# bderembl/msom

Hardware: AMD Instinct MI355X
Metric: grid-point-updates/s (timesteps/s x N^2 x nl), multi-layer QG RK2 step at 4096x4096x6 per GPU (higher is better)
Workload: dtype f64; 1 GPU; C4: msqg double gyre (Verron 1992 params), 4096x4096x6 fp64, tiles 1x1 of 4096x4096, TOLERANCE 1e-3, RK2 step = 2 inversions + 2 tendencies + 2 advances; mg_nrelax=4

## Files before the change

msom_amd/csrc/kernels.h:

```cpp
#ifndef MSOM_KERNELS_H
#define MSOM_KERNELS_H

#include <stdio.h>
#include <stdlib.h>

#include <type_traits>
#include <utility>

#include "msom_internal.h"
#include "modes_inl.h"
#include "floats_inl.h"

template <int LO, int HI, class F>
static inline bool with_int(int v, F &&f) {
  if constexpr (LO > HI) return false;
  else {
    if (v == LO) { f(std::integral_constant<int, LO>{}); return true; }
    return with_int<LO + 1, HI>(v, std::forward<F>(f));
  }
}
template <class F>
static inline void with_bool(bool b, F &&f) {
  if (b) f(std::true_type{});
  else f(std::false_type{});
// ... 180 lines not shown
                        const SplitGeom &sg, int nl, const RelaxCoef &rc, int walls, int nh, int c0, const double *S = nullptr);
void launch_relax_block2(hipStream_t st, const KernelOpts &o, const double *da_in, const double *coarse, const SplitGeom &cg, const double *res, double *da_out,
                         const SplitGeom &sg, int nl, const RelaxCoef &rc, int walls, int fine);
void launch_relax_red_prolong(hipStream_t st, const KernelOpts &o, double *da, const double *coarse, const SplitGeom &cg, const double *res, const double *S,
                              const SplitGeom &sg, int nl, const RelaxCoef &rc, int uniformS, int walls);
void launch_correct(hipStream_t st, double *a, const NatGeom &g, const double *da, const SplitGeom &sg, int nl, int walls);

struct VisitRingBands { int s0[4], ns[4], c0[4], nc[4], n; };
struct MarchCorrect { const double *psi; double *psi_out; NatGeom g; };
struct MarchHalo { const double *in_s, *in_n, *res_s, *res_n; size_t ls; int rows; };
int launch_relax_march(hipStream_t st, const KernelOpts &o, const double *in, double *out, const double *res, const SplitGeom &sg, int nl, const RelaxCoef &rc, int c1,
                       int K, int walls, int chunk_rows = 0, const MarchHalo *h = nullptr, const double *coarse = nullptr, const SplitGeom *cg = nullptr,
                       const MarchCorrect *mc = nullptr, int more_follow = 0, const MarchHalo *coarse_halo = nullptr, int region = 0,
                       const int *skip = nullptr, int skip_compact = 0);
int launch_relax_visit(hipStream_t st, const KernelOpts &o, double *da, double *da_alt, const double *res, const SplitGeom &sg, int nl, const RelaxCoef &rc,
                       int walls, const double *coarse, const SplitGeom &cg, const MarchCorrect &mc);
bool relax_visit_fits(int nl, const SplitGeom &sg, int rows, int pairs);
extern "C" int msom_visit_ring(int hk, int ny, int march_rows, int visit_rows, int pairs, int corr, int *geom, int *bands);
bool march_lean_fits(int nl, const SplitGeom &sg, const NatGeom *ng);

struct ModeCoef {
  double m2l[MSOM_MAXNL * MSOM_MAXNL], ibu[MSOM_MAXNL];
};
int launch_modes_eig(hipStream_t st, const double *S, const NatGeom &g, int nl, int ncx, int ncy, double *out, size_t ols, int per_column,
                     const ModesLayers &l, int *flag);
int launch_modes_get(hipStream_t st, double *out, const double *md, const ModeCoef *mc, const NatGeom &g, int nl, const ModesLayers &l, int which,
                     int first, int cnt);
int launch_modes_rd(hipStream_t st, double *rd, const double *md, const ModeCoef *mc, const NatGeom &g, int nl, int mode);
int launch_modes_project(hipStream_t st, const double *in, double *out, const double *md, const ModeCoef *mc, const NatGeom &g, int nl,
                         const ModesLayers &l, int to_modes);
int modes_energy_blocks(const NatGeom &g);
int modes_energy_stride(const NatGeom &g);
// ... 146 lines not shown
```

msom_amd/csrc/kernels_march.hip:

```cpp
#include <algorithm>
#include <map>
#include <mutex>
#include <type_traits>
#include <utility>
#include "mg_inl.h"
#include "rhs_inl.h"

#pragma clang fp contract(off)

__device__ __forceinline__ double march_rhs(double sqD, double rs, double we, double ns) {
#ifdef MSOM_STRICT
  double v = -sqD * rs;
  v += we;
  v += ns;
  return v;
#else
  return fma(-sqD, rs, we) + ns;
#endif
}
template <int NL>
__device__ __forceinline__ void march_thomas(double (&rhs)[NL], double (&x)[NL], const RelaxCoef &rc) {
#ifdef MSOM_STRICT
#pragma unroll
  for (int l = 1; l < NL; l++) rhs[l] -= rc.w[l] * rhs[l - 1];
// ... 251 lines not shown
            nat_write_ghosts(p.psi_out, p.ng, l, r, 2 * kx, ve, p.walls);
            nat_write_ghosts(p.psi_out, p.ng, l, r, 2 * kx + 1, vo, p.walls);
          }
        }
      }
    }
  }
}

template <int NL, int K, int HL, int WPB, bool PL, bool CORR, int VIS = 0>
struct MarchLeanRows {
  static constexpr int NLE = (NL + 1) & ~1;
  static constexpr int CB = 2 * NLE;
  static constexpr int PBL = (VIS == 2 ? 2 : 3) * NLE;
  static constexpr int XBL = PBL + 2 * NL;
  static constexpr int ROWS = PL ? CB + 4 * NLE : (CORR ? XBL + NL : 3 * NLE);
  static constexpr int RB = PL ? 2 * NLE : 3 * NLE;
  static constexpr int CBD = 2 * RB;
  static constexpr int ROWSD = PL ? CBD + 2 * NLE : 2 * RB;
};

#define MARCH_VMCNT(N) asm volatile("s_waitcnt vmcnt(%0)" ::"n"(N) : "memory")
typedef double v2d __attribute__((ext_vector_type(2)));

template <int NL, int K, int HL, int WPB, bool PL, bool CORR, bool DEEP, int VIS = 0>
__device__ __forceinline__ void march_lean(const MarchArgs &p, double (*ring)[64], const int lane, const int kx0, const int y0, const int y1,
                                           const bool down, double (*hand)[64] = nullptr) {
  static_assert(VIS == 0 || (VIS == 1 && PL && !CORR) || (VIS == 2 && CORR), "fused visit: prolongation leads, correction trails");
  using LR = MarchLeanRows<NL, K, HL, WPB, PL, CORR, VIS>;
  constexpr int D1 = K >= 3 ? 3 : 1, D2 = K >= 4 ? 3 : 1;
  static_assert(!(DEEP && CORR), "no LDS for a second buffer beside the psi block");
  constexpr int NLE = LR::NLE, ND = NLE / 2, CB = DEEP ? LR::CBD : LR::CB, PBL = LR::PBL, XBL = LR::XBL, RB = LR::RB;
  constexpr int CSLOTS = DEEP ? 2 : 4;
  constexpr int NREQ = (PL ? 2 : 3) * ND;
  const int kx = kx0 + lane;
  const bool own_lane = lane >= HL && lane < 64 - HL;
  const int d = down ? -1 : 1;
  const long long rp8 = (long long)p.g.rp * 8, hp8 = (long long)p.g.hp * 8, ls8 = (long long)p.g.ls * 8;
  const long long drp8 = down ? -rp8 : rp8;
  const double sqD = p.rc.sqD;
  const unsigned lds0 = __builtin_amdgcn_readfirstlane((unsigned)(unsigned long long)(__attribute__((address_space(3))) double *)(&ring[0][0]));
  const int sub = lane >> 5;
  unsigned voffL[ND];
// ... 10 lines not shown
      const int la = 2 * q + sub < NL ? 2 * q + sub : NL - 1;
      voffC[q] = (unsigned)(((size_t)la * p.cg.ls + ((lane >> 4) & 1) * p.cg.hp + MSOM_SP + (kx0 >> 1) + 2 * (lane & 15)) * 8);
    }
  }
  const int cld = (lane & 1) * 32 + (lane >> 1);
  const long long crp8 = (long long)p.cg.rp * 8;
  const unsigned voffN = (unsigned)((MSOM_XP + 2 * kx) * 8);
  const long long np8 = (long long)p.ng.pitch * 8, nls8 = (long long)p.ng.ls * 8;
  const long long dnp8 = down ? -np8 : np8;

  const int tA = y0 - K + 1, tB = y1 + K - 2;
  int ra = down ? y0 + y1 - 1 - tA : tA;
  long long rowoff = ((long long)(ra + 1) * p.g.rp + ((ra + p.c1) & 1) * p.g.hp) * 8;
  const char *const res8 = reinterpret_cast<const char *>(p.res);
  const char *const resb8 = res8 - drp8;
  const char *const in8 = PL ? nullptr : reinterpret_cast<const char *>(p.in) + drp8;
  char *const outK8 = CORR ? nullptr : reinterpret_cast<char *>(p.out) - (long long)(K - 1) * drp8;
  long long natoff = CORR ? ((long long)(ra - d * K + MSOM_YP) * p.ng.pitch) * 8 : 0;
  const char *const psi8 = reinterpret_cast<const char *>(p.psi);
  char *const pso8 = reinterpret_cast<char *>(p.psi_out);
  const char *const co8 = reinterpret_cast<const char *>(p.coarse);

  unsigned m0keep;
#define MARCH_DMA(voff, base, ldsrow) \
  asm volatile("s_mov_b32 m0, %2\n\ts_nop 3\n\tglobal_load_lds_dwordx4 %0, %1" ::"v"(voff), "s"(base), "s"(lds0 + (unsigned)(ldsrow) * 512u) : "memory")
  auto request = [&](long long ro, long long no, bool want_psi, int buf = 0) {
    asm volatile("s_mov_b32 %0, m0" : "=s"(m0keep));
    const char *b1 = res8 + ro, *b2 = resb8 + ro;
    const int r0 = buf * RB;
#pragma unroll
    for (int q = 0; q < ND; q++) MARCH_DMA(voffL[q], b1, r0 + 2 * q);
// ... 725 lines not shown
  a.hls = h ? h->ls : 0; a.KR = h ? h->rows : 0;
  a.lean = !o.march_lean ? 0 : o.march_lean * (int)(march_lean_fits(nl, sg, mc ? &mc->g : nullptr) && (!coarse || c1 == 0));
  a.in = in; a.out = out; a.res = res; a.g = sg; a.c1 = c1; a.walls = walls; a.rc = rc; a.remap = o.march_xcd; a.flip = o.march_flip; a.dbg = o.march_dbg;
  if (nl >= 7 && K > 3) return -1;
  int r = -1;
  with_int<1, MSOM_FASTNL>(nl, [&](auto N) { r = march_dispatch<N()>(st, a, K, chunk_rows, o.march_dma); });
  return r;
}

__device__ __forceinline__ void xcd_remap_lin(const unsigned lin, const unsigned nbx, const unsigned total, unsigned &bx, unsigned &by) {
  const unsigned c = lin & 7, q = total >> 3, r = total & 7;
  const unsigned flat = c * q + (c < r ? c : r) + (lin >> 3);
  bx = flat % nbx;
  by = flat / nbx;
}
template <int NL, int PAIRS, int VIS, int KIND>
__device__ __forceinline__ void visit_role(const MarchArgs &p, double (*lds)[64], const int pair) {
  constexpr int K = 4, HL = 8;
  constexpr int OW = 64 - 2 * HL;
  constexpr int RA = MarchLeanRows<NL, K, HL, 2, true, false>::ROWSD, RB = MarchLeanRows<NL, K, HL, 2, false, true, 2>::ROWS;
  const int lane = threadIdx.x & 63;
  unsigned bx = blockIdx.x, by = blockIdx.y;
  if constexpr (KIND != 0) {
    const unsigned lin = blockIdx.x - (unsigned)p.ring_wg;
    if (p.remap) xcd_remap_lin(lin, p.fnbx, (unsigned)p.fnbx * p.fnby, bx, by);
    else { bx = lin % (unsigned)p.fnbx; by = lin / (unsigned)p.fnbx; }
    by += p.fby0;
  } else {
    if (p.remap) xcd_remap(bx, by);
  }
  const int kx0 = p.vx0 + ((int)bx * PAIRS + pair) * OW - HL;
  const int y0 = p.vy0 + (int)by * p.H, y1 = y0 + p.H;
  const bool down = p.flip && (by & 1);
  double(*ring)[64] = lds + pair * (RA + RB + 2 * NL);
  double(*hand)[64] = ring + RA + RB;
  if constexpr (VIS == 2) march_lean<NL, K, HL, 2, false, true, false, 2>(p, ring + RA, lane, kx0, y0, y1, down, hand);
  else march_lean<NL, K, HL, 2, true, false, true, 1>(p, ring, lane, kx0, y0 - K, y1 + K, down, hand);
}
template <int NL, int KIND>
__device__ __forceinline__ void visit_ring_role(const MarchArgs &p, double (*lds)[64], const int wv, const int nwv) {
  constexpr int K = 4;
  const int i = (int)blockIdx.x * nwv + wv;
  if (i >= p.rb.n) return;
  int strip;
  unsigned by;
  visit_ring_chunk(p.rb, i, strip, by);
  MarchArgs q = p;
  q.H = p.rH; q.lean = p.rlean; q.in = p.rin; q.out = p.rout;
  q.partial = KIND == 1;
  q.rb.n = 0; q.region = 0; q.sy0 = q.sy1 = 0;
  const int lane = threadIdx.x & 63;
  if constexpr (KIND == 1) march_dma_chunk<NL, K, 4, 1, true, false>(q, lds + wv * MarchDmaRows<NL, K, 4, 1, true, false>::LROWS, lane, strip, by);
  else march_dma_chunk<NL, K, 2, 1, false, true>(q, lds + wv * MarchDmaRows<NL, K, 2, 1, false, true>::LROWS, lane, strip, by);
}
template <int NL, int PAIRS, int KIND>
__global__ void __launch_bounds__(128 * PAIRS, 2) k_relax_visit(MarchArgs p) {
  constexpr int K = 4, HL = 8;
  constexpr int RA = MarchLeanRows<NL, K, HL, 2, true, false>::ROWSD, RB = MarchLeanRows<NL, K, HL, 2, false, true, 2>::ROWS;
  constexpr int RPL = MarchDmaRows<NL, K, 4, 1, true, false>::LROWS, RCO = MarchDmaRows<NL, K, 2, 1, false, true>::LROWS;
  constexpr int RFUSED = PAIRS * (RA + RB + 2 * NL), RRING = KIND == 0 ? 0 : 2 * PAIRS * (KIND == 1 ? RPL : RCO);
  __shared__ __align__(16) double lds[RFUSED > RRING ? RFUSED : RRING][64];
  const int wv = __builtin_amdgcn_readfirstlane((int)(threadIdx.x >> 6));
  if constexpr (KIND != 0) {
    if ((int)blockIdx.x < p.ring_wg) {
      visit_ring_role<NL, KIND>(p, lds, wv, 2 * PAIRS);
      return;
    }
  }
  if (wv & 1) visit_role<NL, PAIRS, 2, KIND>(p, lds, wv >> 1);
  else visit_role<NL, PAIRS, 1, KIND>(p, lds, wv >> 1);
}

struct VisitGeom { int H, vy0, nc, vx0, ns; };
static bool visit_geom(int hk, int ny, int rows, int pairs, VisitGeom &v) {
  constexpr int K = 4, HL = 8, OW = 64 - 2 * HL;
  v.H = rows > 0 ? (rows + 1) & ~1 : 28;
  v.vy0 = 2 * K;
  v.nc = (ny - 2 * K - v.vy0) / v.H;
  v.vx0 = HL;
  v.ns = hk >= 64 ? ((hk - 64) / OW + 1) / pairs * pairs : 0;
  return v.nc > 0 && v.ns > 0;
}
bool relax_visit_fits(int nl, const SplitGeom &sg, int rows, int pairs) {
  VisitGeom v;
  return nl >= 2 && nl <= 6 && (pairs == 1 || pairs == 2) && visit_geom(sg.hk, sg.ny, rows, pairs, v);
}

static void visit_ring_bands(int hk, int ny, int ow, int H, const int *skip, VisitRingBands &rb) {
  const int ns = (hk + ow - 1) / ow, nc = (ny + H - 1) / H;
  int s_lo = std::min(ns, (std::max(skip[2], 0) + ow - 1) / ow), s_hi = hk <= skip[3] ? ns : std::max(skip[3], 0) / ow;
  int c_lo = std::min(nc, (std::max(skip[0], 0) + H - 1) / H), c_hi = ny <= skip[1] ? nc : std::max(skip[1], 0) / H;
  if (skip[1] <= skip[0] || s_lo >= s_hi || c_lo >= c_hi) { c_lo = c_hi = nc; s_lo = s_hi = ns; }
  const int s0[4] = {0, 0, 0, s_hi}, n_s[4] = {ns, ns, s_lo, ns - s_hi}, c0[4] = {0, c_hi, c_lo, c_lo}, n_c[4] = {c_lo, nc - c_hi, c_hi - c_lo, c_hi - c_lo};
  rb.n = 0;
  for (int b = 0; b < 4; b++) {
    rb.s0[b] = s0[b]; rb.ns[b] = n_s[b]; rb.c0[b] = c0[b]; rb.nc[b] = n_c[b];
    rb.n += n_s[b] * n_c[b];
  }
}
static void visit_skips(const VisitGeom &v, int Hc, int *skip_pl, int *skip_corr) {
// ... 7 lines not shown
extern "C" int msom_visit_ring(int hk, int ny, int march_rows, int visit_rows, int pairs, int corr, int *geom, int *bands) {
  VisitGeom v;
  if (hk <= 0 || ny <= 0 || (pairs != 1 && pairs != 2) || !visit_geom(hk, ny, visit_rows, pairs, v)) return -1;
  int skip_pl[4], skip_corr[4];
  const int Hc = visit_ring_rows(march_rows);
  visit_skips(v, Hc, skip_pl, skip_corr);
  VisitRingBands rb;
  visit_ring_bands(hk, ny, corr ? 60 : 56, Hc, corr ? skip_corr : skip_pl, rb);
  if (geom) { geom[0] = v.H; geom[1] = v.vy0; geom[2] = v.nc; geom[3] = v.vx0; geom[4] = v.ns; }
  if (bands)
    for (int b = 0; b < 4; b++) { bands[b] = rb.s0[b]; bands[4 + b] = rb.ns[b]; bands[8 + b] = rb.c0[b]; bands[12 + b] = rb.nc[b]; }
  return rb.n;
}

template <int NL>
static void visit_dispatch(hipStream_t st, const MarchArgs &a, const VisitGeom &v, int pairs) {
  const dim3 grid = a.ring_kind ? dim3(a.ring_wg + a.fnbx * a.fnby) : dim3(v.ns / pairs, v.nc);
  with_int<0, 2>(a.ring_kind, [&](auto R) {
    with_int<1, 2>(pairs, [&](auto P) {
      constexpr int PAIRS = decltype(P)::value;
      hipLaunchKernelGGL((k_relax_visit<NL, PAIRS, decltype(R)::value>), grid, dim3(128 * PAIRS), 0, st, a);
    });
  });
}
static void visit_dispatch_nl(hipStream_t st, const MarchArgs &a, const VisitGeom &v, int pairs, int nl) {
  if (!with_int<2, 6>(nl, [&](auto N) { visit_dispatch<N()>(st, a, v, pairs); })) no_kernel("launch_relax_visit", nl);
}

int launch_relax_visit(hipStream_t st, const KernelOpts &o, double *da, double *da_alt, const double *res, const SplitGeom &sg, int nl, const RelaxCoef &rc,
                       int walls, const double *coarse, const SplitGeom &cg, const MarchCorrect &mc) {
  const int rows = o.march_visit_rows, pairs = o.march_visit_pairs;
  VisitGeom v;
  if (!relax_visit_fits(nl, sg, rows, pairs)) return -1;
  visit_geom(sg.hk, sg.ny, rows, pairs, v);
  constexpr int K = 4;
  const int Hc = visit_ring_rows(o.march_rows);
  int skip_pl[4], skip_corr[4];
  visit_skips(v, Hc, skip_pl, skip_corr);
  if (o.march_dbg & 16) {
    for (int *s : {skip_pl, skip_corr}) { s[0] = 0; s[1] = sg.ny; s[2] = 0; s[3] = sg.hk; }
  }
  const int ringopt = o.march_visit_ring;
  MarchArgs a{};
  a.res = res; a.g = sg; a.c1 = 0; a.walls = walls; a.rc = rc;
  a.coarse = coarse; a.cg = cg;
  a.psi = mc.psi; a.psi_out = mc.psi_out; a.ng = mc.g;
  a.partial = 1; a.lean = 2;
  a.remap = o.march_xcd; a.flip = o.march_flip;
  a.H = v.H; a.vy0 = v.vy0; a.vx0 = v.vx0;
  if (ringopt >= 2) {
    const int nwv = 2 * pairs;
    a.fnbx = v.ns / pairs;
    a.rH = Hc;
    a.rlean = o.march_lean ? o.march_lean * (int)march_lean_fits(nl, sg, &mc.g) : 0;
    const int n1 = std::min(v.nc, (o.march_visit_split > 0 ? o.march_visit_split : v.nc / 3)) & ~1;
    a.ring_kind = 1;
    visit_ring_bands(sg.hk, sg.ny, 56, Hc, skip_pl, a.rb);
    a.ring_wg = (a.rb.n + nwv - 1) / nwv;
    a.fby0 = 0; a.fnby = n1;
    a.rin = nullptr; a.rout = da_alt;
    visit_dispatch_nl(st, a, v, pairs, nl);
    a.ring_kind = 2;
    visit_ring_bands(sg.hk, sg.ny, 60, Hc, skip_corr, a.rb);
    a.ring_wg = (a.rb.n + nwv - 1) / nwv;
    a.fby0 = n1; a.fnby = v.nc - n1;
    a.rin = da_alt; a.rout = da;
    visit_dispatch_nl(st, a, v, pairs, nl);
    return 0;
  }
  if (launch_relax_march(st, o, nullptr, da_alt, res, sg, nl, rc, 0, K, walls, Hc, nullptr, coarse, &cg, nullptr, 1, nullptr, 0, skip_pl, ringopt == 1)) return -1;
  visit_dispatch_nl(st, a, v, pairs, nl);
  return launch_relax_march(st, o, da_alt, da, res, sg, nl, rc, 0, K, walls, Hc, nullptr, nullptr, nullptr, &mc, 0, nullptr, 0, skip_corr, ringopt == 1);
}
```

msom_amd/csrc/msom_api.hip:

```cpp
#include "msom_host.h"
#include "step_dt_inl.h"

#define RHS_RESID_MIN 23
#define RHS_CLOSE_MIN 23
#define RHS_CLOSE_DEFAULT 2
#define MARCH_HALO 4

static void free_agglomeration(msom *m);

extern "C" const char *msom_version(void) {
#ifdef MSOM_STRICT
  return "msomhip 0.1 (strict: -ffp-contract=off, reference expression order, bit-exact vs oracle)";
#else
  return "msomhip 0.1 (fast: FMA contraction, reciprocal multiplies)";
#endif
}


NatGeom make_nat(int nx, int ny) {
  NatGeom g;
  g.nx = nx; g.ny = ny;
  g.pitch = ((nx + 15) / 16) * 16 + 2 * MSOM_XP;
  g.rows = ny + 2 * MSOM_YP;
  g.ls = (size_t)g.pitch * g.rows;
// ... 456 lines not shown
  else if (!strcmp(key, "uniform_S")) {
    m->uniform_opt = (int)v;
    if (m->const_set) return build_coefs(m);
  }
  else if (!strcmp(key, "profile")) m->profile = (int)v;
  else if (!strcmp(key, "fused")) m->fused = (int)v;
  else if (!strcmp(key, "mg_fused")) m->mg_fused = (int)v;
  else if (!strcmp(key, "march")) m->march = (int)v;
  else if (!strcmp(key, "march_min")) m->march_min = (int)v;
  else if (!strcmp(key, "march_min_tiled")) m->march_min_tiled = (int)v;
  else if (!strcmp(key, "march_partial")) m->march_partial = (int)v;
  else if (!strcmp(key, "march_prolong")) m->march_prolong = (int)v;
  else if (!strcmp(key, "march_correct")) m->march_correct = (int)v;
  else if (!strcmp(key, "march_visit")) m->march_visit = (int)v;
  else if (!strcmp(key, "march_visit_min")) m->march_visit_min = (int)v;
  else if (!strcmp(key, "dbg_nosync")) m->dbg_nosync = (int)v;
  else if (!strcmp(key, "async_solve")) m->async_solve = (int)v;
  else if (!strcmp(key, "step_sync")) m->step_sync = (int)v;
  else if (!strcmp(key, "march_k")) m->march_k = (int)v < 2 ? 2 : ((int)v > 4 ? 4 : (int)v);
  else if (!strcmp(key, "block_small")) m->block_small = (int)v;
  else if (!strcmp(key, "block8")) m->block8 = (int)v;
  else if (!strcmp(key, "restrict2")) m->restrict2 = (int)v;
  else if (!strcmp(key, "restrict_pyr")) m->restrict_pyr = (int)v;
  else if (!strcmp(key, "block8_max")) m->block8_max = (int)v;
  else if (!strcmp(key, "block_sweeps")) { m->block_sweeps = (int)v; if (m->const_set) return build_coefs(m); }
  else if (!strcmp(key, "mg_global_sum")) m->mg_global_sum = (int)v;
  else if (!strcmp(key, "agglomerate")) { m->agglomerate = (int)v; if (m->const_set) return build_coefs(m); }
  else if (!strcmp(key, "agg_size")) { m->agg_size = (int)v; if (m->const_set) return build_coefs(m); }
  else if (!strcmp(key, "prolong_fused")) { m->prolong_fused = (int)v; if (m->const_set) return build_coefs(m); }
  else if (!strcmp(key, "mg_coarse")) { m->mgc_opt = (int)v; if (m->const_set) return build_coefs(m); }
// ... 50 lines not shown
        HIPCHK(hipMalloc(&m->f[k], bytes));
        HIPCHK(hipMemsetAsync(m->f[k], 0, bytes, m->st));
      }
    }
  } else {
    msom_set_error("unknown option %s", key);
    return MSOM_ERR_ARG;
  }
  return MSOM_OK;
}

static int march_levels(const msom *m);
static int march_kmax(const msom *m);
static bool march_lean_fine(const msom *m);
static bool fine_visit_fused(const msom *m);
static int level_path(const msom *m, int k);
static bool restrict2_ok(const msom *m);
static bool rhs_resid_emits(const msom *m, int want = -1);
static int rhs_close_mode(const msom *m);
extern "C" double msom_get_param(msom_t *m, const char *key) {
  if (!m || !key) return NAN;
  if (!strcmp(key, "model")) return m->model;
  if (m->model) return nq_get_param(m, key);
  const Params &p = m->p;
  if (!strcmp(key, "N") || !strcmp(key, "nx")) return m->gnx;
  if (!strcmp(key, "ny")) return m->gny;
  if (!strcmp(key, "nl")) return m->nl;
  if (!strcmp(key, "nptr")) return p.nptr;
  if (!strcmp(key, "L0")) return p.L0;
  if (!strcmp(key, "DT")) return p.DT;
// ... 18 lines not shown
  if (!strcmp(key, "stats_bytes")) {
    int n = m->stats_qme ? 1 : 0;
    for (int k = 0; k < MSOM_ST_NACC; k++) n += m->stats.s[k] ? 1 : 0;
    return (double)n * m->nl * m->nx * m->ny * sizeof(double);
  }
  if (double fv; floats_param(m, key, &fv)) return fv;
  if (!strcmp(key, "mode_pv_invert")) return m->mode_pv_invert;
  if (!strcmp(key, "modes_ready")) return m->const_set && m->modes_ready;
  if (!strcmp(key, "modes_compact")) return m->const_set && m->modes_ready ? m->modes_compact : (m->modes_compact_opt != 0 && m->fr_uniform);
  if (!strcmp(key, "spec_bytes")) return (double)m->spc_bytes;
  if (!strcmp(key, "spec_batch")) return m->spc_batch;
  if (!strcmp(key, "modes_bytes"))
    return m->modes_md ? (double)(m->nl * m->nl + m->nl) * m->nx * m->ny * sizeof(double) : 0.;
  if (!strcmp(key, "resmax_marching")) return m->uniformS && m->nl <= MSOM_FASTNL && m->g.nx >= 64 && m->g.ny >= 16 && m->opt.resmax_rows >= 0;
  if (!strcmp(key, "march_visit_ring")) return !fine_visit_fused(m) ? -1 : (m->opt.march_visit_ring >= 2 ? 2 : (m->opt.march_visit_ring == 1 ? 1 : 0));
  if (const int *o = kernel_opt(m->opt, key)) return *o;
  if (!strcmp(key, "rhs_resid")) return rhs_resid_emits(m);
  if (!strcmp(key, "rhs_close")) return rhs_close_mode(m);
  if (!strncmp(key, "split_ls_", 9)) { const int k = atoi(key + 9); return k >= 0 && k < m->nlev ? (double)m->sg[k].ls : NAN; }
  if (!strncmp(key, "split_rp_", 9)) { const int k = atoi(key + 9); return k >= 0 && k < m->nlev ? (double)m->sg[k].rp : NAN; }
  if (!strcmp(key, "split_pad")) return MSOM_SP;
  if (!strcmp(key, "restrict2")) return restrict2_ok(m);
  if (!strcmp(key, "mg_coarse_lean")) return m->mgc_first >= 0 && m->mgc_lean;
  if (!strcmp(key, "march_levels")) return march_levels(m);
  if (!strcmp(key, "march_min")) return m->march_min;
  if (!strcmp(key, "march_kmax")) return march_kmax(m);
  if (!strcmp(key, "march_lean_fine")) return march_lean_fine(m);
  if (!strcmp(key, "march_visit")) return fine_visit_fused(m);
  if (!strncmp(key, "relax_path_", 11)) { const int k = atoi(key + 11); return k >= 0 && k < m->nlev ? level_path(m, k) : NAN; }
  if (!strcmp(key, "split_ls")) return m->nlev > 0 ? (double)m->sg[0].ls : NAN;
// ... 383 lines not shown
static bool march_lean_fine(const msom *m) {
  return m->nlev > 0 && m->opt.march_lean && level_path(m, 0) == RP_MARCH && march_lean_fits(m->nl, m->sg[0], &m->g);
}
static bool fuse_prolong(const msom *m, const Lev &L, int nrelax) {
  const int path = sweep_path(m, L);
  if (path == RP_BLOCK2 && nrelax >= 2) return true;
  if (path == RP_BLOCK8 && nrelax >= 1) return true;
  return m->prolong_fused && m->nl <= MSOM_FASTNL && nrelax >= 1 && L.sg->nx >= 4 && L.sg->ny >= 4;
}
static bool corr_wanted(const msom *m) { return m->mg_fused && m->nlev > 1 && m->march_correct; }

static int march_kmax(const msom *m) { return m->nl >= 7 && m->march_k > 3 ? 3 : m->march_k; }

enum { MA_DONE, MA_VISIT, MA_PL, MA_REDPROL, MA_PASS, MA_HALF };
struct MarchAct { int kind, K; bool corr, partial; };
static MarchAct march_next(const msom *m, const Lev &L, const Lev *coarse, int n, bool corr_req) {
  const int kmax = march_kmax(m), nl = m->nl;
  const bool deep = L.tiled || (L.walls & WALL_PER);
  auto pass = [&](int kind, int kmin, bool corr_ok) {
    int K = n < kmax ? n : kmax;
    if (n - K == 1 && K > kmin) K--;
    return MarchAct{kind, K, corr_ok && n == K, m->march_partial && n - K >= 1};
  };
  if (coarse && n > 0) {
    const bool pl_tiled = coarse->k >= 0 && nl <= 6 && m->march_prolong >= 1 && coarse->sg->nx >= 2 * MARCH_HALO && coarse->sg->ny >= 2 * MARCH_HALO;
    if (n < 3 || kmax < 3 || !m->march_prolong || (deep && !pl_tiled)) return MarchAct{MA_REDPROL, 1, false, false};
    if (n == 8 && kmax == 4 && L.fine && corr_req && m->march_visit && m->opt.march_dma && m->uniformS && nl >= 2 && m->march_partial &&
        (m->march_visit >= 2 || (size_t)L.sg->nx * L.sg->ny * nl >= ((size_t)1 << m->march_visit_min)) && !L.tiled && L.walls == WALL_ALL &&
        march_lean_fine(m) && relax_visit_fits(nl, *L.sg, m->opt.march_visit_rows, m->opt.march_visit_pairs))
      return MarchAct{MA_VISIT, 8, true, false};
    return pass(MA_PL, 3, false);
  }
  if (n >= 2) return pass(MA_PASS, 2, corr_req && L.fine);
  return MarchAct{n == 1 ? MA_HALF : MA_DONE, n, false, false};
}
static bool fine_visit_fused(const msom *m) {
  if (m->nlev < 2 || level_path(m, 0) != RP_MARCH) return false;
  const Lev L = tile_lev(m, 0), C = tile_lev(m, 1);
  return march_next(m, L, fuse_prolong(m, L, 4) ? &C : nullptr, 8, corr_wanted(m)).kind == MA_VISIT;
}

static bool fine_corr_in_smoother(const msom *m) {
  if (m->nlev < 2 || level_path(m, 0) != RP_MARCH || !corr_wanted(m)) return false;
  const Lev L = tile_lev(m, 0), C = tile_lev(m, 1);
  const Lev *src = fuse_prolong(m, L, 4) ? &C : nullptr;
  for (int n = 8;;) {
    const MarchAct a = march_next(m, L, src, n, true);
    if (a.kind == MA_HALF || a.kind == MA_DONE) return false;
    if (a.kind == MA_VISIT || a.corr) return true;
    src = nullptr; n -= a.K;
  }
}
static bool spec_ok(const msom *m);
// ... 49 lines not shown
      const SplitGeom hgeo = make_split(m->sg[k].nx, MARCH_HALO);
      if (L.tiled) STICKY(m, exch_split_deep(m, f, m->sg[k], fs, fn, hgeo, nl));
      else { launch_split_wrap(m->st, f, m->sg[k], fs, fn, hgeo, nl, MARCH_HALO, 0); launch_split_wrap(m->st, f, m->sg[k], fs, fn, hgeo, nl, MARCH_HALO, 1); }
    };
    MarchHalo mh{nullptr, nullptr, nullptr, nullptr, 0, MARCH_HALO}, ch = mh;
    if (deep && !march_halo(m, L.k, wrap, true, &mh)) return false;
    const bool ovl = L.tiled && m->overlap;
    bool res_halo = deep;
    const MarchCorrect mc{m->f[MSOM_PSI], m->psi_alt, m->g};
    const Lev *src = coarse;
    int n = 2 * nrelax, c = 0;
    for (;;) {
      const MarchAct a = march_next(m, L, src, n, corr_req);
      if (a.kind == MA_HALF || a.kind == MA_DONE) break;
      if (a.kind == MA_VISIT) {
        if (prof) prof_begin(m, m->prof_march_visit);
        if (launch_relax_visit(m->st, m->opt, *L.da, *L.da_alt, L.res, *L.sg, nl, *L.rc, kwalls, *src->da, *src->sg, mc))
          m->sticky = MSOM_ERR_ARG;
        if (prof) prof_end(m, m->prof_march_visit);
        return true;
      } else if (a.kind == MA_REDPROL) {
        if (prof) prof_begin(m, m->prof_redprol);
        launch_relax_red_prolong(m->st, m->opt, *L.da, *src->da, *src->sg, L.res, L.S, *L.sg, nl, *L.rc, m->uniformS, L.walls);
        if (prof) prof_end(m, m->prof_redprol);
      } else {
        const Lev *pl = a.kind == MA_PL ? src : nullptr;
        if (pl && deep && !march_halo(m, pl->k, wrap, false, &ch)) return false;
        march_pass(m, ovl, !prof ? nullptr : (pl ? &m->prof_march_pl : (a.corr ? &m->prof_march_corr : &m->prof_march[a.K])),
                   [&](int region) {
                     if (launch_relax_march(m->st, m->opt, pl ? nullptr : *L.da, *L.da_alt, L.res, *L.sg, nl, *L.rc, c, a.K, kwalls, m->opt.march_rows, deep ? &mh : nullptr,
                                            pl ? *pl->da : nullptr, pl ? pl->sg : nullptr, a.corr ? &mc : nullptr, a.partial, pl && deep ? &ch : nullptr, region))
                       m->sticky = MSOM_ERR_ARG;
                   },
                   [&]() {
                     if (res_halo) fill_halo(L.k, true);
// ... 847 lines not shown
```

msom_amd/csrc/msom_hooks.hip:

```cpp
#include "msom_host.h"


extern "C" int msom_dbg_nlevels(msom_t *m) { return m ? m->nlev : MSOM_ERR_ARG; }
extern "C" int msom_dbg_level_dims(msom_t *m, int lev, int *nx, int *ny) {
  if (!m || lev < 0 || lev >= m->nlev) return MSOM_ERR_ARG;
  *nx = m->sg[lev].nx; *ny = m->sg[lev].ny;
  return MSOM_OK;
}
static int split_upload(msom *m, double *sp, const SplitGeom &sg, const double *a, int nl, int bc) {
  HIPCHK(hipMemcpyAsync(m->staging, a, (size_t)nl * sg.nx * sg.ny * sizeof(double), hipMemcpyDefault, m->st));
  HIPCHK(hipMemsetAsync(sp, 0, sg.ls * nl * sizeof(double), m->st));
  launch_split_pack(m->st, m->staging, sp, sg, nl, bc, m->walls);
  return MSOM_OK;
}
static int split_download(msom *m, const double *sp, const SplitGeom &sg, double *a, int nl) {
  launch_split_unpack(m->st, sp, sg, m->staging, nl);
  HIPCHK(hipMemcpyAsync(a, m->staging, (size_t)nl * sg.nx * sg.ny * sizeof(double), hipMemcpyDefault, m->st));
  return sync_stream(m);
}
extern "C" int msom_dbg_relax(msom_t *m, int lev, double *da, const double *res, int nsweeps) {
  MSQG_ONLY(m);
  if (m) m->res_ready = -1;
  NEED_CONST(m);
  if (lev < 0 || lev >= m->nlev || !da || !res) return MSOM_ERR_ARG;
// ... 123 lines not shown
  else if (!strcmp(op, "stretch")) comp_stretch(m, f_in, f_out, add, fac);
  else if (!strcmp(op, "advection")) {
    launch_advection(m->st, m->f[f_in], m->f[MSOM_PSI], m->f[MSOM_PSIPG], m->f[MSOM_ZETAPG], m->f[MSOM_S], m->f[MSOM_Q], m->f[f_out], m->g,
                     m->nl, m->have_pg, m->have_zpg, m->stochastic, D, p.beta, p.itr_stoch, m->lc);
  } else {
    msom_set_error("unknown op %s", op);
    return MSOM_ERR_ARG;
  }
  return sync_stream(m);
}


std::vector<std::pair<const char *, ProfSlot *>> prof_slots(msom *m) {
  return {{"sweep", &m->prof_sweep}, {"residual", &m->prof_resid}, {"block2", &m->prof_block}, {"march2", &m->prof_march[2]},
          {"march3", &m->prof_march[3]}, {"march4", &m->prof_march[4]}, {"march_pl", &m->prof_march_pl}, {"march_corr", &m->prof_march_corr},
          {"march_visit", &m->prof_march_visit}, {"resid_max", &m->prof_resmax}, {"rhs", &m->prof_rhs}, {"red_prolong", &m->prof_redprol},
          {"resid_correct", &m->prof_rescorr}, {"resid_restrict", &m->prof_respre}, {"helm_relax", &m->prof_helm_relax},
          {"helm_residual", &m->prof_helm_resid}, {"helm_coarse", &m->prof_helm_coarse}, {"floats", &m->prof_floats},
          {"floats_emigrate", &m->prof_floats_emig}, {"floats_immigrate", &m->prof_floats_immig}};
}
extern "C" int msom_profile_reset(msom_t *m) {
  if (!m) return MSOM_ERR_ARG;
  for (const auto &s : prof_slots(m)) { s.second->used = 0; s.second->total_ms = 0; s.second->launches = 0; }
  return MSOM_OK;
}
extern "C" int msom_profile_read(msom_t *m, const char *kernel, double *avg_ms, long *launches) {
  if (!m || !kernel) return MSOM_ERR_ARG;
  ProfSlot *ps = nullptr;
  for (const auto &s : prof_slots(m))
    if (!strcmp(kernel, s.first)) ps = s.second;
  if (!ps) { msom_set_error("unknown kernel %s", kernel); return MSOM_ERR_ARG; }
// ... 106 lines not shown
```

msom_amd/csrc/msom_host.h:

```cpp
#ifndef MSOM_HOST_H
#define MSOM_HOST_H

#include <math.h>
#include <stdio.h>
#include <stdlib.h>
#include <string.h>
#include <sys/stat.h>
#include <sys/types.h>
#include <time.h>

#include <algorithm>
#include <cmath>
#include <string>
#include <utility>
#include <map>
#include <vector>

#include "comm.h"
#include "floats_host.h"
#include "kernels.h"
#include "prof_slot.h"
#include "spec_inl.h"
#include "helm_inl.h"

// ... 70 lines not shown
  int block_sweeps = 0;
  int restrict_pyr = 1;
  int restrict2 = 1;
  int block8 = 1;
  int block8_max = 1024;
  int block_small = 0;
  int march = 1;
  int march_k = 4;
  int use_graph = 0;
  std::map<long, hipGraphExec_t> cyc_graph;
  int march_partial = 1;
  int march_min_tiled = 22;
  int march_min = 23;
  int march_correct = 1;
  int march_visit = 1;
  int march_visit_min = 25;
  int march_prolong = 1;
  int mg_fused = 1;
  double *psi_alt = nullptr;
  int rhs_variant = 6;
  int fused = 1;
  unsigned seed = 1, noise_draw = 0;
  int quiet = 0;
  int wv_nlev = 0, wv_ready = 0;
  int wv_kt = 0, wv_gx = 0, wv_gy = 0;
  std::vector<std::vector<double>> wv_top_sig;
  double *wv_gsend = nullptr, *wv_grecv = nullptr;
  int nme_ft = 0;
  CoarseArgs *d_cargs = nullptr;
  int mgc_dim = MGC_MAXDIM;
  int mgc_pfused = 1;
// ... 51 lines not shown
  NewqgParams nq = {};
  int nq_fused = 1;
  int nq_adv_fused = 1;
  int nq_rows = 0;
  int ckpt_steps = 0, resume = 0;
  long state_flip = -1;
  int run_loaded = 0, run_outdir = 0;
  double run_tout = 0, run_tflt = 0;
  double t = 0, dt = 1., tnext = HUGE_VAL, previous = 0;
  int iter = 0;
  msom_mgstats mg = {0, 0, 0, 0, 0};
  int profile = 0;
  ProfSlot prof_sweep, prof_resid, prof_block, prof_march[5];
  ProfSlot prof_march_pl;
  ProfSlot prof_march_visit;
  ProfSlot prof_march_corr, prof_resmax;
  ProfSlot prof_rhs, prof_redprol, prof_rescorr, prof_respre;
  ProfSlot prof_floats;
  ProfSlot prof_floats_emig, prof_floats_immig;
};

struct RhsPass {
  int qfield, dqfield, with_qforcing;
  int adv_out = -1, adv_in = -1;
  double adv_dt = 0.;
  double *out = nullptr;
  const double *dt_dev = nullptr;
  int cls = 0;
  const double *cls_b = nullptr;
  int emit_resid = -1;
// ... 117 lines not shown
```

Measured before the change: 19.29 billion grid-point-updates/s.

## Extend fused visit relaxation to coarse multigrid levels with auto-tuned row height

Lets the fused prolongation-plus-relaxation visit kernel run on coarse multigrid levels, where it ends in a plain store instead of the psi correction. On coarse levels it replaces separate march passes so fewer kernel launches and memory round trips are needed. It also chooses the visit row height from an occupancy-based slot count when none is set, and lowers the size threshold for the fine-level visit. The new template variant and auto row selection add code paths, and the chosen row height may not suit every grid.

```diff
diff --git a/msom_amd/csrc/kernels.h b/msom_amd/csrc/kernels.h
--- a/msom_amd/csrc/kernels.h
+++ b/msom_amd/csrc/kernels.h
@@ -218,8 +218,10 @@
                        const MarchCorrect *mc = nullptr, int more_follow = 0, const MarchHalo *coarse_halo = nullptr, int region = 0,
                        const int *skip = nullptr, int skip_compact = 0);
 int launch_relax_visit(hipStream_t st, const KernelOpts &o, double *da, double *da_alt, const double *res, const SplitGeom &sg, int nl, const RelaxCoef &rc,
-                       int walls, const double *coarse, const SplitGeom &cg, const MarchCorrect &mc);
+                       int walls, const double *coarse, const SplitGeom &cg, const MarchCorrect *mc);
 bool relax_visit_fits(int nl, const SplitGeom &sg, int rows, int pairs);
+int relax_visit_rows(const KernelOpts &o, int nl, const SplitGeom &sg, bool corr);
+extern "C" int msom_visit_rows(int hk, int ny, int pairs, int slots);
 extern "C" int msom_visit_ring(int hk, int ny, int march_rows, int visit_rows, int pairs, int corr, int *geom, int *bands);
 bool march_lean_fits(int nl, const SplitGeom &sg, const NatGeom *ng);
 
diff --git a/msom_amd/csrc/kernels_march.hip b/msom_amd/csrc/kernels_march.hip
--- a/msom_amd/csrc/kernels_march.hip
+++ b/msom_amd/csrc/kernels_march.hip
@@ -289,7 +289,7 @@
   static constexpr int CB = 2 * NLE;
   static constexpr int PBL = (VIS == 2 ? 2 : 3) * NLE;
   static constexpr int XBL = PBL + 2 * NL;
-  static constexpr int ROWS = PL ? CB + 4 * NLE : (CORR ? XBL + NL : 3 * NLE);
+  static constexpr int ROWS = PL ? CB + 4 * NLE : (CORR ? XBL + NL : (VIS == 2 ? 2 : 3) * NLE);
   static constexpr int RB = PL ? 2 * NLE : 3 * NLE;
   static constexpr int CBD = 2 * RB;
   static constexpr int ROWSD = PL ? CBD + 2 * NLE : 2 * RB;
@@ -301,7 +301,7 @@
 template <int NL, int K, int HL, int WPB, bool PL, bool CORR, bool DEEP, int VIS = 0>
 __device__ __forceinline__ void march_lean(const MarchArgs &p, double (*ring)[64], const int lane, const int kx0, const int y0, const int y1,
                                            const bool down, double (*hand)[64] = nullptr) {
-  static_assert(VIS == 0 || (VIS == 1 && PL && !CORR) || (VIS == 2 && CORR), "fused visit: prolongation leads, correction trails");
+  static_assert(VIS == 0 || (VIS == 1 && PL && !CORR) || (VIS == 2 && !PL && !DEEP), "fused visit: prolongation leads, correction or plain store trails");
   using LR = MarchLeanRows<NL, K, HL, WPB, PL, CORR, VIS>;
   constexpr int D1 = K >= 3 ? 3 : 1, D2 = K >= 4 ? 3 : 1;
   static_assert(!(DEEP && CORR), "no LDS for a second buffer beside the psi block");
@@ -342,7 +342,7 @@
   long long rowoff = ((long long)(ra + 1) * p.g.rp + ((ra + p.c1) & 1) * p.g.hp) * 8;
   const char *const res8 = reinterpret_cast<const char *>(p.res);
   const char *const resb8 = res8 - drp8;
-  const char *const in8 = PL ? nullptr : reinterpret_cast<const char *>(p.in) + drp8;
+  const char *const in8 = PL || VIS == 2 ? nullptr : reinterpret_cast<const char *>(p.in) + drp8;
   char *const outK8 = CORR ? nullptr : reinterpret_cast<char *>(p.out) - (long long)(K - 1) * drp8;
   long long natoff = CORR ? ((long long)(ra - d * K + MSOM_YP) * p.ng.pitch) * 8 : 0;
   const char *const psi8 = reinterpret_cast<const char *>(p.psi);
@@ -1098,11 +1098,11 @@
   bx = flat % nbx;
   by = flat / nbx;
 }
-template <int NL, int PAIRS, int VIS, int KIND>
+template <int NL, int PAIRS, int VIS, int KIND, bool CORR>
 __device__ __forceinline__ void visit_role(const MarchArgs &p, double (*lds)[64], const int pair) {
   constexpr int K = 4, HL = 8;
   constexpr int OW = 64 - 2 * HL;
-  constexpr int RA = MarchLeanRows<NL, K, HL, 2, true, false>::ROWSD, RB = MarchLeanRows<NL, K, HL, 2, false, true, 2>::ROWS;
+  constexpr int RA = MarchLeanRows<NL, K, HL, 2, true, false>::ROWSD, RB = MarchLeanRows<NL, K, HL, 2, false, CORR, 2>::ROWS;
   const int lane = threadIdx.x & 63;
   unsigned bx = blockIdx.x, by = blockIdx.y;
   if constexpr (KIND != 0) {
@@ -1118,10 +1118,10 @@
   const bool down = p.flip && (by & 1);
   double(*ring)[64] = lds + pair * (RA + RB + 2 * NL);
   double(*hand)[64] = ring + RA + RB;
-  if constexpr (VIS == 2) march_lean<NL, K, HL, 2, false, true, false, 2>(p, ring + RA, lane, kx0, y0, y1, down, hand);
+  if constexpr (VIS == 2) march_lean<NL, K, HL, 2, false, CORR, false, 2>(p, ring + RA, lane, kx0, y0, y1, down, hand);
   else march_lean<NL, K, HL, 2, true, false, true, 1>(p, ring, lane, kx0, y0 - K, y1 + K, down, hand);
 }
-template <int NL, int KIND>
+template <int NL, int KIND, bool CORR>
 __device__ __forceinline__ void visit_ring_role(const MarchArgs &p, double (*lds)[64], const int wv, const int nwv) {
   constexpr int K = 4;
   const int i = (int)blockIdx.x * nwv + wv;
@@ -1135,24 +1135,24 @@
   q.rb.n = 0; q.region = 0; q.sy0 = q.sy1 = 0;
   const int lane = threadIdx.x & 63;
   if constexpr (KIND == 1) march_dma_chunk<NL, K, 4, 1, true, false>(q, lds + wv * MarchDmaRows<NL, K, 4, 1, true, false>::LROWS, lane, strip, by);
-  else march_dma_chunk<NL, K, 2, 1, false, true>(q, lds + wv * MarchDmaRows<NL, K, 2, 1, false, true>::LROWS, lane, strip, by);
-}
-template <int NL, int PAIRS, int KIND>
+  else march_dma_chunk<NL, K, 2, 1, false, CORR>(q, lds + wv * MarchDmaRows<NL, K, 2, 1, false, CORR>::LROWS, lane, strip, by);
+}
+template <int NL, int PAIRS, int KIND, bool CORR = true>
 __global__ void __launch_bounds__(128 * PAIRS, 2) k_relax_visit(MarchArgs p) {
   constexpr int K = 4, HL = 8;
-  constexpr int RA = MarchLeanRows<NL, K, HL, 2, true, false>::ROWSD, RB = MarchLeanRows<NL, K, HL, 2, false, true, 2>::ROWS;
-  constexpr int RPL = MarchDmaRows<NL, K, 4, 1, true, false>::LROWS, RCO = MarchDmaRows<NL, K, 2, 1, false, true>::LROWS;
+  constexpr int RA = MarchLeanRows<NL, K, HL, 2, true, false>::ROWSD, RB = MarchLeanRows<NL, K, HL, 2, false, CORR, 2>::ROWS;
+  constexpr int RPL = MarchDmaRows<NL, K, 4, 1, true, false>::LROWS, RCO = MarchDmaRows<NL, K, 2, 1, false, CORR>::LROWS;
   constexpr int RFUSED = PAIRS * (RA + RB + 2 * NL), RRING = KIND == 0 ? 0 : 2 * PAIRS * (KIND == 1 ? RPL : RCO);
   __shared__ __align__(16) double lds[RFUSED > RRING ? RFUSED : RRING][64];
   const int wv = __builtin_amdgcn_readfirstlane((int)(threadIdx.x >> 6));
   if constexpr (KIND != 0) {
     if ((int)blockIdx.x < p.ring_wg) {
-      visit_ring_role<NL, KIND>(p, lds, wv, 2 * PAIRS);
+      visit_ring_role<NL, KIND, CORR>(p, lds, wv, 2 * PAIRS);
       return;
     }
   }
-  if (wv & 1) visit_role<NL, PAIRS, 2, KIND>(p, lds, wv >> 1);
-  else visit_role<NL, PAIRS, 1, KIND>(p, lds, wv >> 1);
+  if (wv & 1) visit_role<NL, PAIRS, 2, KIND, CORR>(p, lds, wv >> 1);
+  else visit_role<NL, PAIRS, 1, KIND, CORR>(p, lds, wv >> 1);
 }
 
 struct VisitGeom { int H, vy0, nc, vx0, ns; };
@@ -1165,9 +1165,30 @@
   v.ns = hk >= 64 ? ((hk - 64) / OW + 1) / pairs * pairs : 0;
   return v.nc > 0 && v.ns > 0;
 }
+static int visit_rows_auto(int hk, int ny, int pairs, int slots) {
+  constexpr int K = 4;
+  VisitGeom v;
+  const bool fits28 = visit_geom(hk, ny, 28, pairs, v);
+  if (slots <= 0) return fits28 ? 28 : 14;
+  if (fits28 && (long long)v.nc * v.ns > 3LL * slots) return 28;
+  int best = 14;
+  long long cost = -1;
+  for (int H = 14; H <= ny; H += 2) {
+    if (!visit_geom(hk, ny, H, pairs, v)) break;
+    const long long c = (((long long)v.nc * v.ns + slots - 1) / slots) * (H + 4 * K - 1);
+    if (cost < 0 || c < cost) { cost = c; best = H; }
+  }
+  return best;
+}
+extern "C" int msom_visit_rows(int hk, int ny, int pairs, int slots) {
+  if (hk <= 0 || ny <= 0 || (pairs != 1 && pairs != 2)) return -1;
+  VisitGeom v;
+  const int H = visit_rows_auto(hk, ny, pairs, slots);
+  return visit_geom(hk, ny, H, pairs, v) ? H : -1;
+}
 bool relax_visit_fits(int nl, const SplitGeom &sg, int rows, int pairs) {
   VisitGeom v;
-  return nl >= 2 && nl <= 6 && (pairs == 1 || pairs == 2) && visit_geom(sg.hk, sg.ny, rows, pairs, v);
+  return nl >= 2 && nl <= 6 && (pairs == 1 || pairs == 2) && visit_geom(sg.hk, sg.ny, rows > 0 ? rows : 14, pairs, v);
 }
 
 static void visit_ring_bands(int hk, int ny, int ow, int H, const int *skip, VisitRingBands &rb) {
@@ -1205,25 +1226,64 @@
 }
 
 template <int NL>
-static void visit_dispatch(hipStream_t st, const MarchArgs &a, const VisitGeom &v, int pairs) {
+static void visit_dispatch(hipStream_t st, const MarchArgs &a, const VisitGeom &v, int pairs, bool corr) {
   const dim3 grid = a.ring_kind ? dim3(a.ring_wg + a.fnbx * a.fnby) : dim3(v.ns / pairs, v.nc);
+  if (!grid.x || !grid.y) return;
   with_int<0, 2>(a.ring_kind, [&](auto R) {
     with_int<1, 2>(pairs, [&](auto P) {
       constexpr int PAIRS = decltype(P)::value;
-      hipLaunchKernelGGL((k_relax_visit<NL, PAIRS, decltype(R)::value>), grid, dim3(128 * PAIRS), 0, st, a);
+      if (corr) hipLaunchKernelGGL((k_relax_visit<NL, PAIRS, decltype(R)::value, true>), grid, dim3(128 * PAIRS), 0, st, a);
+      else hipLaunchKernelGGL((k_relax_visit<NL, PAIRS, decltype(R)::value, false>), grid, dim3(128 * PAIRS), 0, st, a);
     });
   });
 }
-static void visit_dispatch_nl(hipStream_t st, const MarchArgs &a, const VisitGeom &v, int pairs, int nl) {
-  if (!with_int<2, 6>(nl, [&](auto N) { visit_dispatch<N()>(st, a, v, pairs); })) no_kernel("launch_relax_visit", nl);
+static void visit_dispatch_nl(hipStream_t st, const MarchArgs &a, const VisitGeom &v, int pairs, int nl, bool corr) {
+  if (!with_int<2, 6>(nl, [&](auto N) { visit_dispatch<N()>(st, a, v, pairs, corr); })) no_kernel("launch_relax_visit", nl);
+}
+static int visit_slots(int nl, int pairs, int kind, bool corr) {
+  const void *kern = nullptr;
+  with_int<2, 6>(nl, [&](auto N) {
+    with_int<0, 2>(kind, [&](auto R) {
+      with_int<1, 2>(pairs, [&](auto P) {
+        constexpr int NL = decltype(N)::value, PAIRS = decltype(P)::value, KIND = decltype(R)::value;
+        kern = corr ? (const void *)k_relax_visit<NL, PAIRS, KIND, true> : (const void *)k_relax_visit<NL, PAIRS, KIND, false>;
+      });
+    });
+  });
+  if (!kern) return 0;
+  static std::mutex mu;
+  static std::map<std::pair<int, const void *>, int> cache;
+  int dev = 0;
+  (void)hipGetDevice(&dev);
+  int per_cu = 0;
+  {
+    std::lock_guard<std::mutex> lock(mu);
+    auto it = cache.find({dev, kern});
+    if (it == cache.end()) {
+      if (hipOccupancyMaxActiveBlocksPerMultiprocessor(&per_cu, kern, 128 * pairs, 0) != hipSuccess || per_cu <= 0) per_cu = 4 / pairs;
+      cache[{dev, kern}] = per_cu;
+    } else {
+      per_cu = it->second;
+    }
+  }
+  return per_cu * pairs * device_cu_count();
+}
+int relax_visit_rows(const KernelOpts &o, int nl, const SplitGeom &sg, bool corr) {
+  if (o.march_visit_rows > 0) return (o.march_visit_rows + 1) & ~1;
+  const int pairs = o.march_visit_pairs;
+  if (nl < 2 || nl > 6 || (pairs != 1 && pairs != 2)) return 0;
+  const int slots = o.march_visit_ring >= 2 ? std::min(visit_slots(nl, pairs, 1, corr), visit_slots(nl, pairs, 2, corr)) : visit_slots(nl, pairs, 0, corr);
+  return visit_rows_auto(sg.hk, sg.ny, pairs, slots);
 }
 
 int launch_relax_visit(hipStream_t st, const KernelOpts &o, double *da, double *da_alt, const double *res, const SplitGeom &sg, int nl, const RelaxCoef &rc,
-                       int walls, const double *coarse, const SplitGeom &cg, const MarchCorrect &mc) {
-  const int rows = o.march_visit_rows, pairs = o.march_visit_pairs;
+                       int walls, const double *coarse, const SplitGeom &cg, const MarchCorrect *mc) {
+  const int pairs = o.march_visit_pairs;
+  const bool corr = mc != nullptr;
   VisitGeom v;
-  if (!relax_visit_fits(nl, sg, rows, pairs)) return -1;
-  visit_geom(sg.hk, sg.ny, rows, pairs, v);
+  if (!relax_visit_fits(nl, sg, o.march_visit_rows, pairs)) return -1;
+  const int rows = relax_visit_rows(o, nl, sg, corr);
+  if (!visit_geom(sg.hk, sg.ny, rows, pairs, v)) return -1;
   constexpr int K = 4;
   const int Hc = visit_ring_rows(o.march_rows);
   int skip_pl[4], skip_corr[4];
@@ -1235,31 +1295,32 @@
   MarchArgs a{};
   a.res = res; a.g = sg; a.c1 = 0; a.walls = walls; a.rc = rc;
   a.coarse = coarse; a.cg = cg;
-  a.psi = mc.psi; a.psi_out = mc.psi_out; a.ng = mc.g;
-  a.partial = 1; a.lean = 2;
+  if (mc) { a.psi = mc->psi; a.psi_out = mc->psi_out; a.ng = mc->g; }
+  a.partial = corr ? 1 : 0; a.lean = 2;
+  a.out = corr ? nullptr : da;
   a.remap = o.march_xcd; a.flip = o.march_flip;
   a.H = v.H; a.vy0 = v.vy0; a.vx0 = v.vx0;
   if (ringopt >= 2) {
     const int nwv = 2 * pairs;
     a.fnbx = v.ns / pairs;
     a.rH = Hc;
-    a.rlean = o.march_lean ? o.march_lean * (int)march_lean_fits(nl, sg, &mc.g) : 0;
-    const int n1 = std::min(v.nc, (o.march_visit_split > 0 ? o.march_visit_split : v.nc / 3)) & ~1;
+    a.rlean = o.march_lean ? o.march_lean * (int)march_lean_fits(nl, sg, mc ? &mc->g : nullptr) : 0;
+    const int n1 = o.march_visit_split < 0 ? 0 : std::min(v.nc, (o.march_visit_split > 0 ? o.march_visit_split : v.nc / 3)) & ~1;
     a.ring_kind = 1;
     visit_ring_bands(sg.hk, sg.ny, 56, Hc, skip_pl, a.rb);
     a.ring_wg = (a.rb.n + nwv - 1) / nwv;
     a.fby0 = 0; a.fnby = n1;
     a.rin = nullptr; a.rout = da_alt;
-    visit_dispatch_nl(st, a, v, pairs, nl);
+    visit_dispatch_nl(st, a, v, pairs, nl, corr);
     a.ring_kind = 2;
     visit_ring_bands(sg.hk, sg.ny, 60, Hc, skip_corr, a.rb);
     a.ring_wg = (a.rb.n + nwv - 1) / nwv;
     a.fby0 = n1; a.fnby = v.nc - n1;
     a.rin = da_alt; a.rout = da;
-    visit_dispatch_nl(st, a, v, pairs, nl);
+    visit_dispatch_nl(st, a, v, pairs, nl, corr);
     return 0;
   }
   if (launch_relax_march(st, o, nullptr, da_alt, res, sg, nl, rc, 0, K, walls, Hc, nullptr, coarse, &cg, nullptr, 1, nullptr, 0, skip_pl, ringopt == 1)) return -1;
-  visit_dispatch_nl(st, a, v, pairs, nl);
-  return launch_relax_march(st, o, da_alt, da, res, sg, nl, rc, 0, K, walls, Hc, nullptr, nullptr, nullptr, &mc, 0, nullptr, 0, skip_corr, ringopt == 1);
-}
+  visit_dispatch_nl(st, a, v, pairs, nl, corr);
+  return launch_relax_march(st, o, da_alt, da, res, sg, nl, rc, 0, K, walls, Hc, nullptr, nullptr, nullptr, mc, 0, nullptr, 0, skip_corr, ringopt == 1);
+}
diff --git a/msom_amd/csrc/msom_api.hip b/msom_amd/csrc/msom_api.hip
--- a/msom_amd/csrc/msom_api.hip
+++ b/msom_amd/csrc/msom_api.hip
@@ -4,6 +4,8 @@
 #define RHS_RESID_MIN 23
 #define RHS_CLOSE_MIN 23
 #define RHS_CLOSE_DEFAULT 2
+#define MARCH_VISIT_LEVELS_DEFAULT 1
+#define MARCH_VISIT_LEVELS_MIN 23
 #define MARCH_HALO 4
 
 static void free_agglomeration(msom *m);
@@ -494,6 +496,7 @@
   else if (!strcmp(key, "march_correct")) m->march_correct = (int)v;
   else if (!strcmp(key, "march_visit")) m->march_visit = (int)v;
   else if (!strcmp(key, "march_visit_min")) m->march_visit_min = (int)v;
+  else if (!strcmp(key, "march_visit_levels")) m->march_visit_levels = (int)v;
   else if (!strcmp(key, "dbg_nosync")) m->dbg_nosync = (int)v;
   else if (!strcmp(key, "async_solve")) m->async_solve = (int)v;
   else if (!strcmp(key, "step_sync")) m->step_sync = (int)v;
@@ -574,6 +577,7 @@
 static int march_kmax(const msom *m);
 static bool march_lean_fine(const msom *m);
 static bool fine_visit_fused(const msom *m);
+static bool level_visit_fused(const msom *m, int k);
 static int level_path(const msom *m, int k);
 static bool restrict2_ok(const msom *m);
 static bool rhs_resid_emits(const msom *m, int want = -1);
@@ -622,6 +626,12 @@
     return m->modes_md ? (double)(m->nl * m->nl + m->nl) * m->nx * m->ny * sizeof(double) : 0.;
   if (!strcmp(key, "resmax_marching")) return m->uniformS && m->nl <= MSOM_FASTNL && m->g.nx >= 64 && m->g.ny >= 16 && m->opt.resmax_rows >= 0;
   if (!strcmp(key, "march_visit_ring")) return !fine_visit_fused(m) ? -1 : (m->opt.march_visit_ring >= 2 ? 2 : (m->opt.march_visit_ring == 1 ? 1 : 0));
+  if (!strncmp(key, "march_visit_rows_", 17) && key[17] >= '0' && key[17] <= '9') {
+    const int k = atoi(key + 17);
+    return level_visit_fused(m, k) ? relax_visit_rows(m->opt, m->nl, m->sg[k], k == 0) : 0;
+  }
+  if (!strncmp(key, "march_visit_", 12) && key[12] >= '0' && key[12] <= '9') return level_visit_fused(m, atoi(key + 12));
+  if (!strcmp(key, "march_visit_levels")) return m->march_visit_levels;
   if (const int *o = kernel_opt(m->opt, key)) return *o;
   if (!strcmp(key, "rhs_resid")) return rhs_resid_emits(m);
   if (!strcmp(key, "rhs_close")) return rhs_close_mode(m);
@@ -1035,6 +1045,10 @@
 
 enum { MA_DONE, MA_VISIT, MA_PL, MA_REDPROL, MA_PASS, MA_HALF };
 struct MarchAct { int kind, K; bool corr, partial; };
+static bool visit_levels_on(const msom *m, const Lev &L) {
+  if (m->march_visit_levels >= 0) return m->march_visit_levels > 0;
+  return MARCH_VISIT_LEVELS_DEFAULT && (size_t)L.sg->nx * L.sg->ny * m->nl >= ((size_t)1 << MARCH_VISIT_LEVELS_MIN);
+}
 static MarchAct march_next(const msom *m, const Lev &L, const Lev *coarse, int n, bool corr_req) {
   const int kmax = march_kmax(m), nl = m->nl;
   const bool deep = L.tiled || (L.walls & WALL_PER);
@@ -1050,6 +1064,10 @@
         (m->march_visit >= 2 || (size_t)L.sg->nx * L.sg->ny * nl >= ((size_t)1 << m->march_visit_min)) && !L.tiled && L.walls == WALL_ALL &&
         march_lean_fine(m) && relax_visit_fits(nl, *L.sg, m->opt.march_visit_rows, m->opt.march_visit_pairs))
       return MarchAct{MA_VISIT, 8, true, false};
+    if (n == 8 && kmax == 4 && !L.fine && L.k > 0 && visit_levels_on(m, L) && m->opt.march_dma && m->uniformS && nl >= 2 && m->march_partial &&
+        !L.tiled && L.walls == WALL_ALL && m->opt.march_lean && march_lean_fits(nl, *L.sg, nullptr) &&
+        relax_visit_fits(nl, *L.sg, m->opt.march_visit_rows, m->opt.march_visit_pairs))
+      return MarchAct{MA_VISIT, 8, false, false};
     return pass(MA_PL, 3, false);
   }
   if (n >= 2) return pass(MA_PASS, 2, corr_req && L.fine);
@@ -1058,6 +1076,12 @@
 static bool fine_visit_fused(const msom *m) {
   if (m->nlev < 2 || level_path(m, 0) != RP_MARCH) return false;
   const Lev L = tile_lev(m, 0), C = tile_lev(m, 1);
+  return march_next(m, L, fuse_prolong(m, L, 4) ? &C : nullptr, 8, corr_wanted(m)).kind == MA_VISIT;
+}
+static bool level_visit_fused(const msom *m, int k) {
+  if (k == 0) return fine_visit_fused(m);
+  if (k < 0 || k + 1 >= m->nlev || level_path(m, k) != RP_MARCH) return false;
+  const Lev L = tile_lev(m, k), C = tile_lev(m, k + 1);
   return march_next(m, L, fuse_prolong(m, L, 4) ? &C : nullptr, 8, corr_wanted(m)).kind == MA_VISIT;
 }
 
@@ -1137,11 +1161,12 @@
       const MarchAct a = march_next(m, L, src, n, corr_req);
       if (a.kind == MA_HALF || a.kind == MA_DONE) break;
       if (a.kind == MA_VISIT) {
-        if (prof) prof_begin(m, m->prof_march_visit);
-        if (launch_relax_visit(m->st, m->opt, *L.da, *L.da_alt, L.res, *L.sg, nl, *L.rc, kwalls, *src->da, *src->sg, mc))
+        ProfSlot *ps = !m->profile ? nullptr : (a.corr ? &m->prof_march_visit : &m->prof_march_visit_coarse);
+        if (ps) prof_begin(m, *ps);
+        if (launch_relax_visit(m->st, m->opt, *L.da, *L.da_alt, L.res, *L.sg, nl, *L.rc, kwalls, *src->da, *src->sg, a.corr ? &mc : nullptr))
           m->sticky = MSOM_ERR_ARG;
-        if (prof) prof_end(m, m->prof_march_visit);
-        return true;
+        if (ps) prof_end(m, *ps);
+        return a.corr;
       } else if (a.kind == MA_REDPROL) {
         if (prof) prof_begin(m, m->prof_redprol);
         launch_relax_red_prolong(m->st, m->opt, *L.da, *src->da, *src->sg, L.res, L.S, *L.sg, nl, *L.rc, m->uniformS, L.walls);
diff --git a/msom_amd/csrc/msom_hooks.hip b/msom_amd/csrc/msom_hooks.hip
--- a/msom_amd/csrc/msom_hooks.hip
+++ b/msom_amd/csrc/msom_hooks.hip
@@ -161,7 +161,7 @@
 std::vector<std::pair<const char *, ProfSlot *>> prof_slots(msom *m) {
   return {{"sweep", &m->prof_sweep}, {"residual", &m->prof_resid}, {"block2", &m->prof_block}, {"march2", &m->prof_march[2]},
           {"march3", &m->prof_march[3]}, {"march4", &m->prof_march[4]}, {"march_pl", &m->prof_march_pl}, {"march_corr", &m->prof_march_corr},
-          {"march_visit", &m->prof_march_visit}, {"resid_max", &m->prof_resmax}, {"rhs", &m->prof_rhs}, {"red_prolong", &m->prof_redprol},
+          {"march_visit", &m->prof_march_visit}, {"march_visit_coarse", &m->prof_march_visit_coarse}, {"resid_max", &m->prof_resmax}, {"rhs", &m->prof_rhs}, {"red_prolong", &m->prof_redprol},
           {"resid_correct", &m->prof_rescorr}, {"resid_restrict", &m->prof_respre}, {"helm_relax", &m->prof_helm_relax},
           {"helm_residual", &m->prof_helm_resid}, {"helm_coarse", &m->prof_helm_coarse}, {"floats", &m->prof_floats},
           {"floats_emigrate", &m->prof_floats_emig}, {"floats_immigrate", &m->prof_floats_immig}};
diff --git a/msom_amd/csrc/msom_host.h b/msom_amd/csrc/msom_host.h
--- a/msom_amd/csrc/msom_host.h
+++ b/msom_amd/csrc/msom_host.h
@@ -108,7 +108,8 @@
   int march_min = 23;
   int march_correct = 1;
   int march_visit = 1;
-  int march_visit_min = 25;
+  int march_visit_min = 23;
+  int march_visit_levels = -1;
   int march_prolong = 1;
   int mg_fused = 1;
   double *psi_alt = nullptr;
@@ -190,6 +191,7 @@
   ProfSlot prof_sweep, prof_resid, prof_block, prof_march[5];
   ProfSlot prof_march_pl;
   ProfSlot prof_march_visit;
+  ProfSlot prof_march_visit_coarse;
   ProfSlot prof_march_corr, prof_resmax;
   ProfSlot prof_rhs, prof_redprol, prof_rescorr, prof_respre;
   ProfSlot prof_floats;
```

Result: faster. 20.06 billion grid-point-updates/s (median of 6 runs) (+4.0%).
